# vidify/old-audiosync

Measured on NVIDIA B200. Metric: xcorr_pairs_per_sec_L1440000, higher is better.
Workload: dtype f32

## Files before the change

### old-audiosync_b200/csrc/fft_kernels.cuh

```cuda
#pragma once

#include "common.cuh"
#include "fft_device.cuh"

namespace asc {

constexpr int COL_T = 16;

constexpr int ctas_per_sm(size_t smem, int threads) {
    const int by_smem = (int)((228u * 1024u) / (smem + 1024u));
    const int by_threads = 1024 / threads;
    const int n = by_smem < by_threads ? by_smem : by_threads;
    return n >= 3 ? 3 : (n >= 1 ? n : 1);
}
constexpr unsigned TW2_BITS = 10;
constexpr unsigned TW2_MASK = (1u << TW2_BITS) - 1u;

template <class C>
ASC_HD C tw2(const C* __restrict__ lo, const C* __restrict__ hi, unsigned a) {
    return cmul(ldg(lo + (a & TW2_MASK)), ldg(hi + (a >> TW2_BITS)));
}

constexpr int tile_boxes(int rows) { return (rows + 255) / 256; }
constexpr int tile_box_rows(int rows) { return (rows + tile_boxes(rows) - 1) / tile_boxes(rows); }
constexpr int tile_box_start(int rows, int i) {
    return i * tile_box_rows(rows) + tile_box_rows(rows) <= rows ? i * tile_box_rows(rows) : rows - tile_box_rows(rows);
}

template <typename InT>
ASC_HD cplx load_packed(const InT* __restrict__ x, long long n, bool vec = true);

template <>
ASC_HD cplx load_packed<float>(const float* __restrict__ x, long long n, bool) {
    return ldg(reinterpret_cast<const float2*>(x) + n);
}
template <>
ASC_HD cplx load_packed<double>(const double* __restrict__ x, long long n, bool) {
    double2 d = ldg(reinterpret_cast<const double2*>(x) + n);
    return cmake(in_real<float>(d.x), in_real<float>(d.y));
}
template <>
ASC_HD cplx load_packed<int16_t>(const int16_t* __restrict__ x, long long n, bool vec) {
    if (vec) {
        const short2 s = ldg(reinterpret_cast<const short2*>(x) + n);
        return cmake(in_real<float>(s.x), in_real<float>(s.y));
    }
    return cmake(in_real<float>(ldg(x + 2 * n)), in_real<float>(ldg(x + 2 * n + 1)));
}

struct ArgmaxPair {
    unsigned long long best;
    float second;
};

struct ArgmaxAcc {
    unsigned long long best = 0ull;
    float second = 0.0f;
    float thr = 0.0f;
    ASC_HD void update(unsigned long long key, float a) {
        if (key > best) {
            if (best != 0ull && !argmax_key_is_seed(best)) second = fmaxf(second, argmax_key_mag(best));
            best = key;
        } else {
            second = fmaxf(second, a);
        }
        thr = fmaxf(thr, second);
    }
    ASC_HD void consider(float v, uint32_t index) {
        const float a = fabsf(v);
        if (a >= thr) update(argmax_key_abs(v, index), a);
    }
    ASC_HD void consider_seed(float v, PairPeak* pk) {
        update(argmax_key_seed(v), 0.0f);
        pk->seed_bits = float_order_bits(fabsf(v));
    }
    ASC_HD float best_mag() const { return best != 0ull && !argmax_key_is_seed(best) ? argmax_key_mag(best) : 0.0f; }
    ASC_HD ArgmaxPair result() const { ArgmaxPair r; r.best = best; r.second = second; return r; }
};

ASC_HD void argmax_merge(unsigned long long& best, float& second, unsigned long long ob, float os) {
    const unsigned long long lose = ob > best ? best : ob;
    best = ob > best ? ob : best;
    second = fmaxf(second, os);
    if (lose != 0ull && !argmax_key_is_seed(lose)) second = fmaxf(second, argmax_key_mag(lose));
}

template <class RL, int M2_, int NT, typename InT, bool TMA>
struct ColFwdKernel {
    static constexpr int M1 = RL::n;
    static constexpr int M2 = M2_;
    static constexpr int P = RL::count;
    static constexpr int THREADS = NT;
    static constexpr size_t SMEM = (size_t)M1 * COL_T * sizeof(cplx);
    static constexpr int MIN_CTAS = ctas_per_sm(SMEM, NT);
    static_assert(NT % COL_T == 0, "a thread must keep its column across items");
    static_assert(P >= 2, "column plans need at least two passes");
    static_assert(!TMA || std::is_same<InT, float>::value, "TMA staging copies packed fp32 pairs verbatim");
    static_assert(!TMA || M1 >= 4, "tile too small for a box");
    static_assert(M1 % 2 == 0, "the zero half of the sample must be whole tile rows");

    struct Params {
        const InT* sources;
        const InT* samples;
        cplx* planes;
        PairPeak* peaks;
        const cplx* tw;
        const cplx* tc;
        const cplx* m_lo;
        const cplx* m_hi;
        long long L;
        long long src_pitch;
        long long smp_pitch;
        int vec_src, vec_smp;
        CUtensorMap tm_src, tm_smp;
    };
    static constexpr int SRC_ROWS = M1 - 1, SMP_ROWS = M1 / 2;

    template <class Ex>
    static ASC_HD void run(Ex& ex, const Params& p, cplx* __restrict__ buf) {
        const int c0 = ex.bx() * COL_T;
        const int sig = ex.by();
        const long long pair = ex.bz();
        const long long M = p.L;
        const InT* __restrict__ x = sig == 0 ? p.sources + pair * (p.src_pitch ? p.src_pitch : 2 * M)
                                             : p.samples + pair * (p.smp_pitch ? p.smp_pitch : M);
        const long long nvalid = sig == 0 ? M : M / 2;
        [[maybe_unused]] const bool vec = sig == 0 ? p.vec_src != 0 : p.vec_smp != 0;
        cplx* __restrict__ out = p.planes + (pair * 2 + sig) * M;
        const bool clears_peak = ex.bx() == 0 && sig == 0;

        [[maybe_unused]] void* mbar = reinterpret_cast<char*>(buf) + SMEM - 8;
        if constexpr (TMA) {
            ex.phase([&](int tid) {
                if (tid == 0) {
                    if (clears_peak) p.peaks[pair] = cleared_peak();
                    mbar_init(mbar, 1);
                }
            });
            ex.phase([&](int tid) {
                if (tid == 0) {
                    const char* __restrict__ raw = reinterpret_cast<const char*>(x) + (size_t)c0 * sizeof(cplx);
                    constexpr size_t pitch = (size_t)M2 * sizeof(cplx);
                    if (sig == 0) {
                        constexpr int NB = tile_boxes(SRC_ROWS), BR = tile_box_rows(SRC_ROWS);
                        mbar_expect_tx(mbar, (unsigned)(NB * BR * 128));
                        static_for<0, NB>([&](auto I) {
                            constexpr int r0 = tile_box_start(SRC_ROWS, decltype(I)::value);
                            tma_load_rows(buf + r0 * COL_T, &p.tm_src, 2 * c0, r0, (int)pair, mbar, raw + r0 * pitch, pitch, BR);
                        });
                    } else {
                        constexpr int NB = tile_boxes(SMP_ROWS), BR = tile_box_rows(SMP_ROWS);
                        mbar_expect_tx(mbar, (unsigned)(NB * BR * 128));
                        static_for<0, NB>([&](auto I) {
                            constexpr int r0 = tile_box_start(SMP_ROWS, decltype(I)::value);
                            tma_load_rows(buf + r0 * COL_T, &p.tm_smp, 2 * c0, r0, (int)pair, mbar, raw + r0 * pitch, pitch, BR);
                        });
                    }
                }
                mbar_wait(mbar, 0);
            });
        }

        static_for<0, P>([&](auto PP) {
            constexpr int ps = decltype(PP)::value;
            constexpr int R = RL::r(ps);
            constexpr int S = RL::stride(ps);
            constexpr bool first = ps == 0, last = ps == P - 1;
            constexpr bool from_global = first && !TMA;
            constexpr int items = (M1 / R) * COL_T;
            ex.phase([&](int tid) {
                if (from_global && clears_peak && tid == 0) p.peaks[pair] = cleared_peak();
                const int c = tid & (COL_T - 1);
                if constexpr (!last) {
                    auto items_loop = [&](auto HZ) {
                        [[maybe_unused]] constexpr bool hz = decltype(HZ)::value;
                        cplx t[R];
                        for (int w = tid; w < items; w += NT) {
                            const int bf = w >> 4;
                            const int blk = (S * R == M1) ? 0 : bf / S;
                            const int j = bf - blk * S;
                            const int i0 = blk * (S * R) + j;
                            cplx v[R];
                            if constexpr (from_global) {
                                static_for<0, R>([&](auto Q) {
                                    constexpr int q = decltype(Q)::value;
                                    const long long n = (long long)(i0 + q * S) * M2 + c0 + c;
                                    v[q] = n < nvalid ? load_packed<InT>(x, n, vec) : cmake(0.f, 0.f);
                                });
                            } else {
                                static_for<0, R>([&](auto Q) {
                                    constexpr int q = decltype(Q)::value;
                                    if constexpr (hz && 2 * q >= R) {
                                        v[q] = cmake(0.f, 0.f);
                                    } else if constexpr (TMA && first && !hz && q == R - 1) {
                                        if (i0 == S - 1) v[q] = load_packed<InT>(x, (long long)(M1 - 1) * M2 + c0 + c);
                                        else v[q] = buf[(i0 + q * S) * COL_T + c];
                                    } else {
                                        v[q] = buf[(i0 + q * S) * COL_T + c];
                                    }
                                });
                                if constexpr (TMA && first) {
                                    if (i0 == S - 1 && c == COL_T - 1) mbar_inval(mbar);
                                }
                            }
                            dft_reg<R, -1>(v);
                            pass_twiddles<R>(p.tw + RL::tw_offset(ps), S, j, t);
                            buf[i0 * COL_T + c] = v[0];
                            static_for<1, R>([&](auto K) {
                                constexpr int k = decltype(K)::value;
                                buf[(i0 + k * S) * COL_T + c] = cmul(v[k], t[k]);
                            });
                        }
                    };
                    if constexpr (first && TMA) {
                        static_assert(R % 2 == 0 && S * R == M1, "zero-pad rows must be the inputs q >= R/2 of pass 0");
                        if (sig == 1) items_loop(std::true_type{});
                        else items_loop(std::false_type{});
                    } else {
                        items_loop(std::false_type{});
                    }
                } else {
                    constexpr int Wt = RL::weight(ps);
                    const unsigned n2 = (unsigned)(c0 + c);
                    constexpr bool lean_g = R > 8;
                    cplx g[R];
                    if constexpr (!lean_g) {
                        static_assert(R <= 8, "power chain written for k < 8");
                        g[1] = tw2(p.m_lo, p.m_hi, n2 * (unsigned)Wt);
                        static_for<2, R>([&](auto K) {
                            constexpr int k = decltype(K)::value;
                            g[k] = (k % 2 == 0) ? cmul(g[k / 2], g[k / 2]) : cmul(g[k - 1], g[1]);
                        });
                    } else {
                        static_for<1, R>([&](auto K) {
                            constexpr int k = decltype(K)::value;
                            if constexpr (!lean_g || (k & (k - 1)) == 0)
                                g[k] = tw2(p.m_lo, p.m_hi, n2 * (unsigned)(Wt * k));
                        });
                    }
                    constexpr int ITER = (items + NT - 1) / NT;
                    constexpr int CH = ITER <= 6 ? ITER : 4;
                    constexpr int DB = NT / COL_T, UNIT = RL::stride(0) / R;
                    constexpr bool STEP = ITER > 1 && DB % UNIT == 0;
                    constexpr int MSTEP = STEP ? DB / UNIT : 0;
                    [[maybe_unused]] int f0_run = 0;
                    [[maybe_unused]] cplx t0_run = cmake(1.f, 0.f), gstep = cmake(1.f, 0.f);
                    if constexpr (STEP) {
                        f0_run = RL::freq_of_pos(((tid < items ? tid : 0) >> 4) * R);
                        t0_run = cmul(ldg(p.tc + f0_run * COL_T + c), tw2(p.m_lo, p.m_hi, (unsigned)c0 * (unsigned)f0_run));
                        gstep = tw2(p.m_lo, p.m_hi, n2 * (unsigned)MSTEP);
                    }
                    for (int it0 = 0; it0 < ITER; it0 += CH) {
                        int f0s[CH];
                        cplx t0s[CH];
                        static_for<0, CH>([&](auto I) {
                            constexpr int i = decltype(I)::value;
                            if constexpr (STEP) {
                                f0s[i] = f0_run;
                                t0s[i] = t0_run;
                                f0_run += MSTEP;
                                t0_run = cmul(t0_run, gstep);
                            } else {
                                const int w = tid + (it0 + i) * NT;
                                f0s[i] = RL::freq_of_pos(((w < items ? w : 0) >> 4) * R);
                                t0s[i] = cmul(ldg(p.tc + f0s[i] * COL_T + c),
                                              tw2(p.m_lo, p.m_hi, (unsigned)c0 * (unsigned)f0s[i]));
                            }
                        });
                        static_for<0, CH>([&](auto I) {
                            constexpr int i = decltype(I)::value;
                            const int w = tid + (it0 + i) * NT;
                            if (w < items) {
                                const int i0 = (w >> 4) * R;
                                cplx v[R];
                                static_for<0, R>([&](auto Q) {
                                    constexpr int q = decltype(Q)::value;
                                    v[q] = buf[(i0 + q) * COL_T + c];
                                });
                                dft_reg<R, -1>(v);
                                const cplx t0 = t0s[i];
                                cplx* __restrict__ o = out + ((unsigned)f0s[i] * (unsigned)M2 + n2);
                                o[0] = cmul(v[0], t0);
                                static_for<1, R>([&](auto K) {
                                    constexpr int k = decltype(K)::value;
                                    cplx gk;
                                    if constexpr (!lean_g || (k & (k - 1)) == 0) {
                                        gk = g[k];
                                    } else {
                                        constexpr int hb = (k >= 16) ? 16 : (k >= 8) ? 8 : (k >= 4) ? 4 : 2;
                                        constexpr int rest = k - hb;
                                        if constexpr ((rest & (rest - 1)) == 0) {
                                            gk = cmul(g[hb], g[rest]);
                                        } else {
                                            constexpr int hb2 = (rest >= 8) ? 8 : (rest >= 4) ? 4 : 2;
                                            constexpr int rest2 = rest - hb2;
                                            static_assert(R <= 24, "k < 24: at most four one-bits, and then the last two are 2 + 1");
                                            if constexpr ((rest2 & (rest2 - 1)) == 0) gk = cmul(g[hb], cmul(g[hb2], g[rest2]));
                                            else gk = cmul(cmul(g[hb], g[hb2]), cmul(g[rest2 & ~1], g[1]));
                                        }
                                    }
                                    o[(size_t)k * Wt * M2] = cmul(v[k], cmul(t0, gk));
                                });
                            }
                        });
                    }
                }
            });
        });
    }
};

template <class RL, int M2_, int NT, bool TMA = true>
struct ColInvKernel {
    static_assert(TMA, "K_C's tiles are always staged by the TMA unit");
    static constexpr int M1 = RL::n;
    static constexpr int M2 = M2_;
    static constexpr int P = RL::count;
    static constexpr int THREADS = NT;
    static constexpr size_t SMEM = (size_t)M1 * COL_T * sizeof(cplx);
    static constexpr int MIN_CTAS = ctas_per_sm(SMEM, NT);
    static_assert(NT % COL_T == 0, "a thread must keep its column across items");
    static_assert(NT % 32 == 0, "the argmax epilogue votes per warp");
    static_assert(P >= 2, "column plans need at least two passes");

    struct Params {
        const cplx* planes;
        PairPeak* peaks;
        const cplx* tw;
        long long L;
        CUtensorMap tm;
    };
    static constexpr int TMA_ROWS = M1 - 1;

    template <class Ex>
    static ASC_HD void run(Ex& ex, const Params& p, cplx* __restrict__ buf) {
        const int c0 = ex.by() * COL_T;
        const long long pair = ex.bx();
        const long long M = p.L;
        const cplx* __restrict__ in = p.planes + pair * 2 * M;

        void* mbar = reinterpret_cast<char*>(buf) + SMEM - 8;
        ex.phase([&](int tid) {
            if (tid == 0) mbar_init(mbar, 1);
        });
        ex.phase([&](int tid) {
            if (tid == 0) {
                constexpr int NB = tile_boxes(TMA_ROWS), BR = tile_box_rows(TMA_ROWS);
                constexpr size_t pitch = (size_t)M2 * sizeof(cplx);
                const char* __restrict__ raw = reinterpret_cast<const char*>(in + c0);
                mbar_expect_tx(mbar, (unsigned)(NB * BR * 128));
                static_for<0, NB>([&](auto I) {
                    constexpr int r0 = tile_box_start(TMA_ROWS, decltype(I)::value);
                    tma_load_rows(buf + r0 * COL_T, &p.tm, 2 * c0, r0, (int)(2 * pair), mbar, raw + r0 * pitch, pitch, BR);
                });
            }
            mbar_wait(mbar, 0);
        });

        static_for<0, P - 1>([&](auto PP) {
            constexpr int ps = decltype(PP)::value;
            constexpr int R = RL::r(ps);
            constexpr int S = RL::stride(ps);
            constexpr int items = (M1 / R) * COL_T;
            ex.phase([&](int tid) {
                const int c = tid & (COL_T - 1);
                cplx t[R];
                for (int w = tid; w < items; w += NT) {
                    const int bf = w >> 4;
                    const int blk = (S * R == M1) ? 0 : bf / S;
                    const int j = bf - blk * S;
                    const int i0 = blk * (S * R) + j;
                    cplx v[R];
                    static_for<0, R>([&](auto Q) {
                        constexpr int q = decltype(Q)::value;
                        if constexpr (ps == 0 && q == R - 1) {
                            if (i0 == S - 1) v[q] = ldg(in + ((long long)(M1 - 1) * M2 + c0 + c));
                            else v[q] = buf[(i0 + q * S) * COL_T + c];
                        } else {
                            v[q] = buf[(i0 + q * S) * COL_T + c];
                        }
                    });
                    if constexpr (ps == 0) {
                        if (i0 == S - 1 && c == COL_T - 1) mbar_inval(mbar);
                    }
                    dft_reg<R, +1>(v);
                    pass_twiddles<R>(p.tw + RL::tw_offset(ps), S, j, t);
                    buf[i0 * COL_T + c] = v[0];
                    static_for<1, R>([&](auto K) {
                        constexpr int k = decltype(K)::value;
                        buf[(i0 + k * S) * COL_T + c] = cmulc(v[k], t[k]);
                    });
                }
            });
        });

        {
            constexpr int ps = P - 1;
            constexpr int R = RL::r(ps);
            constexpr int Wt = RL::weight(ps);
            constexpr int items = (M1 / R) * COL_T;
            ex.phase_argmax(
                [&](int tid) -> ArgmaxPair {
                    ArgmaxAcc acc;
                    const unsigned int seen = ex.peek_bits(&p.peaks[pair].second_bits);
                    if (seen != 0u) acc.thr = float_from_order_bits(seen);
                    const int c = tid & (COL_T - 1);
                    const bool col0 = (c0 + c) == 0;
                    for (int w0 = 0; w0 < items; w0 += NT) {
                        const int w = w0 + tid;
                        const bool act = w < items;
                        const int blk = (act ? w : 0) >> 4;
                        const int i0 = blk * R;
                        cplx v[R];
                        static_for<0, R>([&](auto Q) {
                            constexpr int q = decltype(Q)::value;
                            v[q] = buf[(i0 + q) * COL_T + c];
                        });
                        dft_reg<R, +1>(v);
                        float gm = fmaxf(fabsf(v[0].x), fabsf(v[0].y));
                        static_for<1, R>([&](auto K) {
                            constexpr int k = decltype(K)::value;
                            gm = fmaxf(gm, fmaxf(fabsf(v[k].x), fabsf(v[k].y)));
                        });
                        const bool has_seed = col0 && i0 == 0;
                        const bool need = act && (gm >= acc.thr || has_seed);
                        if (ex.any(need)) {
                            if (need) {
                                const int f0 = RL::freq_of_pos(i0);
                                static_for<0, R>([&](auto K) {
                                    constexpr int k = decltype(K)::value;
                                    const int n1 = f0 + k * Wt;
                                    const uint32_t i_re = 2u * ((uint32_t)n1 * (uint32_t)M2 + (uint32_t)(c0 + c));
                                    if (has_seed && n1 == 0) acc.consider_seed(v[k].x, &p.peaks[pair]);
                                    else acc.consider(v[k].x, i_re);
                                    acc.consider(v[k].y, i_re + 1u);
                                });
                            }
                            acc.thr = fmaxf(acc.thr, ex.warp_second(acc.best_mag(), acc.second));
                        }
                    }
                    return acc.result();
                },
                &p.peaks[pair].key, &p.peaks[pair].second_bits, buf);
        }
    }
};

ASC_HD void split_mul_merge(cplx a, cplx b, cplx c, cplx d, cplx w, cplx& qk, cplx& qmk) {
    const cplx s = cmake(a.x + b.x, a.y - b.y);
    const cplx t = cmake(a.x - b.x, a.y + b.y);
    const cplx u = cmul(w, cmake(t.y, -t.x));
    const cplx s2 = cmake(c.x + d.x, c.y - d.y);
    const cplx t2 = cmake(c.x - d.x, c.y + d.y);
    const cplx u2 = cmul(w, cmake(t2.y, -t2.x));
    const cplx p1 = cmulc(cadd(s, u), cadd(s2, u2));
    const cplx p2 = cmulc(csub(s, u), csub(s2, u2));
    const cplx g = cadd(p1, p2);
    const cplx e = csub(p1, p2);
    const cplx ce = cmulc(e, w);
    const cplx h = cmake(-ce.y, ce.x);
    qk = cmake(0.25f * (g.x + h.x), 0.25f * (g.y + h.y));
    qmk = cmake(0.25f * (g.x - h.x), -0.25f * (g.y - h.y));
}

template <class C>
ASC_HD void split_mul_merge_w2(C a, C b, C c, C d, C w2, C& qk2, C& qmk2) {
    const C s = cconj_add(a, b), t = cconj_sub(a, b);
    const C s2 = cconj_add(c, d), t2 = cconj_sub(c, d);
    const C g = cmulc_acc(t, t2, cmulc(s, s2));
    const C x = cmulc(s, t2);
    const C h = cmulc_nacc(x, w2, cmulc(t, s2));
    qk2 = cadd(g, h);
    const C e = csub(g, h);
    qmk2 = cmake(e.x, -e.y);
}

ASC_HD float phat_rsqrt(float q) {
#if defined(__CUDA_ARCH__)
    return rsqrtf(q);
#else
    return 1.0f / sqrtf(q);
#endif
}
ASC_HD double phat_rsqrt(double q) {
#if defined(__CUDA_ARCH__)
    return rsqrt(q);
#else
    return 1.0 / sqrt(q);
#endif
}
ASC_HD cplx unit_phasor(cplx z) {
    const float m = fmaxf(fabsf(z.x), fabsf(z.y));
    uint32_t b;
    memcpy(&b, &m, 4);
    int e = (int)(b >> 23);
    e = e < 1 ? 1 : (e > 253 ? 253 : e);
    const uint32_t sb = (uint32_t)(254 - e) << 23;
    float s;
    memcpy(&s, &sb, 4);
    const float x = z.x * s, y = z.y * s;
    const float q = fmaf(x, x, y * y);
    const float r = q > 0.0f ? phat_rsqrt(q) : 0.0f;
    return cmake(x * r, y * r);
}
ASC_HD cplxd unit_phasor(cplxd z) {
    const double m = fmax(fabs(z.x), fabs(z.y));
    uint64_t b;
    memcpy(&b, &m, 8);
    int e = (int)(b >> 52);
    e = e < 1 ? 1 : (e > 2045 ? 2045 : e);
    const uint64_t sb = (uint64_t)(2046 - e) << 52;
    double s;
    memcpy(&s, &sb, 8);
    const double x = z.x * s, y = z.y * s;
    const double q = fma(x, x, y * y);
    const double r = q > 0.0 ? phat_rsqrt(q) : 0.0;
    return cmake(x * r, y * r);
}

template <int SCALE, class C>
ASC_HD void split_phat_merge(C a, C b, C c, C d, C w, C& qk, C& qmk) {
    static_assert(SCALE == 1 || SCALE == 2, "output convention of split_mul_merge or split_mul_merge_w2");
    const C s = cconj_add(a, b), t = cconj_sub(a, b);
    const C s2 = cconj_add(c, d), t2 = cconj_sub(c, d);
    const C u = cmul_ni(cmul(w, t)), u2 = cmul_ni(cmul(w, t2));
    const C p1 = cmulc(unit_phasor(cadd(s, u)), unit_phasor(cadd(s2, u2)));
    const C p2 = cmulc(unit_phasor(csub(s, u)), unit_phasor(csub(s2, u2)));
    C g = cadd(p1, p2);
    C h = cmul_pi(cmulc(csub(p1, p2), w));
    if constexpr (SCALE == 2) {
        g = cadd(g, g);
        h = cadd(h, h);
    }
    qk = cadd(g, h);
    const C e = csub(g, h);
    qmk = cmake(e.x, -e.y);
}

template <class RL, int M1_, int NT, bool PHAT = false>
struct RowFusedKernel {
    static constexpr int M2 = RL::n;
    static constexpr int M1 = M1_;
    static constexpr int P = RL::count;
    static constexpr int THREADS = NT;
    static constexpr int RP = M2;
    static constexpr size_t SMEM = (size_t)4 * RP * sizeof(cplx);
    static constexpr int MIN_CTAS = ctas_per_sm(SMEM, NT);
    static constexpr int R0 = RL::r(0);
    static constexpr int S0 = RL::stride(0);
    static_assert(M2 % 2 == 0, "row length must be even (16-byte chunks, bulk store size)");
    static_assert(P >= 2, "row plans need at least two passes");
    static_assert(S0 * R0 == M2 && S0 >= 16, "pass 0 must own the last two points of a row as its last two items");

    static constexpr int slots(int S) { return (S > 1 && S < 16) ? 16 : S; }

    struct Params {
        cplx* planes;
        const cplx* tw;
        const cplx* rev;
        const cplx* m_lo;
        const cplx* m_hi;
        long long L;
        const cplx* rtab;
        int m1 = 0;
    };
    static constexpr int TABP = (S0 + R0 + 1) & ~1;
    static_assert(NT % 64 == 0, "the split phase maps threads to an (NT/64) x 64 grid");
    static constexpr int SPLIT_A = NT / 64;
    static constexpr int SPLIT_XN = (R0 + SPLIT_A - 1) / SPLIT_A;
    static constexpr int SPLIT_MN = (S0 + 63) / 64;
    static_assert(2 * TABP + 1 <= 2 * RP, "final-pass twiddle tables and their mbarrier must fit the dead sample rows");

    template <class Ex>
    static ASC_HD void run(Ex& ex, const Params& p, cplx* __restrict__ buf) {
        const int r = ex.bx();
        const long long pair = ex.bz();
        const long long M = p.L;
        const int m1 = M1 > 0 ? M1 : p.m1;
        const bool two = (r != 0) && (2 * r != m1);
        const int nrows = two ? 2 : 1;
        const int k1a = r, k1b = m1 - r;
        cplx* __restrict__ plane_s = p.planes + pair * 2 * M;
        cplx* __restrict__ plane_p = plane_s + M;
        cplx* __restrict__ tab = buf + 2 * RP;
        void* tabbar = buf + 2 * RP + 2 * TABP;

        {
            void* mbar = buf + 4 * RP - 1;
            ex.phase([&](int tid) {
                if (tid == 0) mbar_init(mbar, 1);
            });
            ex.phase([&](int tid) {
                if (tid == 0) {
                    constexpr unsigned full = (unsigned)(M2 * sizeof(cplx));
                    mbar_expect_tx(mbar, two ? 4u * full - 16u : 2u * full);
                    bulk_load(buf, plane_s + (long long)k1a * M2, full, mbar);
                    bulk_load(buf + 2 * RP, plane_p + (long long)k1a * M2, full, mbar);
                    if (two) {
                        bulk_load(buf + RP, plane_s + (long long)k1b * M2, full, mbar);
                        bulk_load(buf + 3 * RP, plane_p + (long long)k1b * M2, full - 16u, mbar);
                    }
                }
                mbar_wait(mbar, 0);
            });
        }

        auto fwd_pass = [&](auto PP, int t, int nt, int slot0, int sstep, int nb) {
            constexpr int ps = decltype(PP)::value;
            constexpr int R = RL::r(ps);
            constexpr int S = RL::stride(ps);
            constexpr int SL = slots(S);
            constexpr int per_row = (M2 / (S * R)) * SL;
            const int items = per_row * nb;
            [[maybe_unused]] const int tail_w = (slot0 + (nb - 1) * sstep == 3) ? items - 2 : 0x7fffffff;
            {
                for (int w = t; w < items; w += nt) {
                    const int bw = w / per_row;
                    const int bf = w - bw * per_row;
                    const int blk = (per_row == SL) ? 0 : bf / SL;
                    const int j = bf - blk * SL;
                    if (SL != S && j >= S) continue;
                    cplx* __restrict__ row = buf + (slot0 + bw * sstep) * RP;
                    const int i0 = blk * (S * R) + j;
                    cplx v[R];
                    static_for<0, R>([&](auto Q) {
                        constexpr int q = decltype(Q)::value;
                        v[q] = row[i0 + q * S];
                    });
                    if constexpr (ps == 0) {
                        if (w >= tail_w) {
                            v[R - 1] = ldg(plane_p + (long long)k1b * M2 + (i0 + (R - 1) * S));
                            if (w == tail_w + 1) mbar_inval(buf + 4 * RP - 1);
                        }
                    }
                    dft_reg<R, -1>(v);
                    row[i0] = v[0];
                    if constexpr (S > 1) {
                        cplx t[R];
                        pass_twiddles<R>(p.tw + RL::tw_offset(ps), S, j, t);
                        static_for<1, R>([&](auto K) {
                            constexpr int k = decltype(K)::value;
                            row[i0 + k * S] = cmul(v[k], t[k]);
                        });
                    } else {
                        static_for<1, R>([&](auto K) {
                            constexpr int k = decltype(K)::value;
                            row[i0 + k] = v[k];
                        });
                    }
                }
            }
        };
        static_for<0, P>([&](auto PP) {
            ex.phase([&](int tid) { fwd_pass(PP, tid, NT, 0, two ? 1 : 2, 2 * nrows); });
        });

        {
            ex.phase([&](int tid) {
                const cplx wk1 = tw2(p.m_lo, p.m_hi, (unsigned)k1a);
                if (two) {
                    cplx* __restrict__ zs_a = buf;
                    cplx* __restrict__ zs_b = buf + RP;
                    cplx* __restrict__ zp_a = buf + 2 * RP;
                    cplx* __restrict__ zp_b = buf + 3 * RP;
                    cplx ax[SPLIT_XN], cm[SPLIT_MN];
                    const int sa = tid >> 6, sb = tid & 63;
                    static_for<0, SPLIT_XN>([&](auto X) {
                        const int d0 = sa + decltype(X)::value * SPLIT_A;
                        ax[decltype(X)::value] = cmul(ldg(p.rev + (d0 < R0 ? d0 : 0) * S0), wk1);
                    });
                    static_for<0, SPLIT_MN>([&](auto Mm) {
                        const int e1 = sb + decltype(Mm)::value * 64;
                        cm[decltype(Mm)::value] = ldg(p.rev + (e1 < S0 ? e1 : 0));
                    });
                    static_for<0, SPLIT_MN>([&](auto Mm) {
#if defined(__CUDA_ARCH__)
                        if constexpr (decltype(Mm)::value > 0 && decltype(Mm)::value % 2 == 0)
                            asm volatile("" ::: "memory");
#endif
                        static_for<0, SPLIT_XN>([&](auto X) {
                            const int d0 = sa + decltype(X)::value * SPLIT_A;
                            const int e1 = sb + decltype(Mm)::value * 64;
                            if (d0 < R0 && e1 < S0) {
                                const int e = d0 * S0 + e1;
                                const int pb = M2 - 1 - e;
                                const cplx w2 = cmul(ax[decltype(X)::value], cm[decltype(Mm)::value]);
                                cplx qk, qmk;
                                if constexpr (PHAT) split_phat_merge<2>(zs_a[e], zs_b[pb], zp_a[e], zp_b[pb], w2, qk, qmk);
                                else split_mul_merge_w2(zs_a[e], zs_b[pb], zp_a[e], zp_b[pb], w2, qk, qmk);
                                zs_a[e] = qk;
                                zs_b[pb] = qmk;
                            }
                        });
                    });
                } else {
                    cplx* __restrict__ zs = buf;
                    cplx* __restrict__ zp = buf + 2 * RP;
                    const int items = r == 0 ? M2 / 2 + 1 : M2 / 2;
                    for (int e = tid; e < items; e += NT) {
                        int pa, pb;
                        if (r == 0) {
                            pa = RL::pos_of_freq(e);
                            pb = RL::pos_of_freq(e == 0 ? 0 : M2 - e);
                        } else {
                            pa = e;
                            pb = M2 - 1 - e;
                        }
                        const cplx w2 = cmul(ldg(p.rev + pa), wk1);
                        cplx qk, qmk;
                        if constexpr (PHAT) split_phat_merge<2>(zs[pa], zs[pb], zp[pa], zp[pb], w2, qk, qmk);
                        else split_mul_merge_w2(zs[pa], zs[pb], zp[pa], zp[pb], w2, qk, qmk);
                        zs[pa] = qk;
                        if (pa != pb) zs[pb] = qmk;
                    }
                }
            });
        }

        ex.single([&]() {
            constexpr unsigned bytes = (unsigned)(TABP * sizeof(cplx));
            mbar_init(tabbar, 1);
            mbar_expect_tx(tabbar, (unsigned)nrows * bytes);
            bulk_load(tab, p.rtab + (long long)k1a * TABP, bytes, tabbar);
            if (two) bulk_load(tab + TABP, p.rtab + (long long)k1b * TABP, bytes, tabbar);
        });

        auto inv_pass = [&](auto PP, int t, int nt, int r0, int nr) {
            constexpr int ps = P - 1 - decltype(PP)::value;
            constexpr int R = RL::r(ps);
            constexpr int S = RL::stride(ps);
            constexpr int SL = slots(S);
            constexpr bool last = ps == 0;
            constexpr int per_row = (M2 / (S * R)) * SL;
            const int items = per_row * nr;
            {
                if constexpr (last) mbar_wait(tabbar, 0);
                for (int w = t; w < items; w += nt) {
                    const int rw = w / per_row;
                    const int rr = r0 + rw;
                    const int bf = w - rw * per_row;
                    const int blk = (per_row == SL) ? 0 : bf / SL;
                    const int j = bf - blk * SL;
                    if (SL != S && j >= S) continue;
                    cplx* __restrict__ row = buf + rr * RP;
                    const int i0 = blk * (S * R) + j;
                    cplx v[R];
                    v[0] = row[i0];
                    if constexpr (S > 1) {
                        cplx t[R];
                        pass_twiddles<R>(p.tw + RL::tw_offset(ps), S, j, t);
                        static_for<1, R>([&](auto Q) {
                            constexpr int q = decltype(Q)::value;
                            v[q] = cmulc(row[i0 + q * S], t[q]);
                        });
                    } else {
                        static_for<1, R>([&](auto Q) {
                            constexpr int q = decltype(Q)::value;
                            v[q] = row[i0 + q];
                        });
                    }
                    dft_reg<R, +1>(v);
                    if constexpr (!last) {
                        static_for<0, R>([&](auto K) {
                            constexpr int k = decltype(K)::value;
                            row[i0 + k * S] = v[k];
                        });
                    } else {
                        const cplx t0 = tab[rr * TABP + j];
                        row[j] = cmulc(v[0], t0);
                        static_for<1, R>([&](auto K) {
                            constexpr int k = decltype(K)::value;
                            row[j + k * S] = cmulc(v[k], cmul(t0, tab[rr * TABP + S0 + k]));
                        });
                    }
                }
                if constexpr (last) fence_async_proxy();
            }
        };
        static_for<0, P>([&](auto PP) {
            ex.phase([&](int tid) { inv_pass(PP, tid, NT, 0, nrows); });
        });

        ex.single([&]() {
            bulk_store(plane_s + (long long)k1a * M2, buf, (unsigned)(M2 * sizeof(cplx)));
            if (two) bulk_store(plane_s + (long long)k1b * M2, buf + RP, (unsigned)(M2 * sizeof(cplx)));
            bulk_store_commit_and_drain();
        });
    }
};

struct DeviceExec {
    int x_ = 0, y_ = 0, z_ = 0;
    ASC_HD int bx() const { return x_; }
    ASC_HD int by() const { return y_; }
    ASC_HD int bz() const { return z_; }
    template <class F>
    ASC_HD void phase(F&& f) {
#if defined(__CUDA_ARCH__)
        f((int)threadIdx.x);
        __syncthreads();
#endif
    }
    template <class F>
    ASC_HD void single(F&& f) {
#if defined(__CUDA_ARCH__)
        if (threadIdx.x == 0) f();
#endif
    }
    ASC_HD bool any(bool b) const {
#if defined(__CUDA_ARCH__)
        return __any_sync(0xffffffffu, b);
#else
        return b;
#endif
    }
    ASC_HD float warp_second(float best_mag, float second) const {
#if defined(__CUDA_ARCH__)
        const unsigned bm = __float_as_uint(fmaxf(best_mag, 0.0f));
        const unsigned top = __reduce_max_sync(0xffffffffu, bm);
        const unsigned holders = __ballot_sync(0xffffffffu, bm == top);
        const bool winner = (threadIdx.x & 31u) == (unsigned)(__ffs(holders) - 1);
        const float cand = winner ? second : fmaxf(second, best_mag);
        return __uint_as_float(__reduce_max_sync(0xffffffffu, __float_as_uint(fmaxf(cand, 0.0f))));
#else
        (void)best_mag;
        return second;
#endif
    }
    ASC_HD unsigned long long peek_key(const unsigned long long* k) const {
#if defined(__CUDA_ARCH__)
        return __ldcg(k);
#else
        return *k;
#endif
    }
    ASC_HD unsigned int peek_bits(const unsigned int* k) const {
#if defined(__CUDA_ARCH__)
        return __ldcg(k);
#else
        return *k;
#endif
    }
    template <class F>
    ASC_HD void phase_argmax(F&& f, unsigned long long* dst, unsigned int* dst_second, void* scratch) {
#if defined(__CUDA_ARCH__)
        unsigned long long* s_best = reinterpret_cast<unsigned long long*>(scratch);
        float* s_sec = reinterpret_cast<float*>(s_best + 32);
        const ArgmaxPair mine = f((int)threadIdx.x);
        unsigned long long best = mine.best;
        float second = mine.second;
        for (int o = 16; o > 0; o >>= 1)
            argmax_merge(best, second, __shfl_xor_sync(0xffffffffu, best, o), __shfl_xor_sync(0xffffffffu, second, o));
        const int wid = threadIdx.x >> 5, lane = threadIdx.x & 31;
        const int nw = (blockDim.x + 31) >> 5;
        __syncthreads();
        if (lane == 0) { s_best[wid] = best; s_sec[wid] = second; }
        __syncthreads();
        if (wid == 0) {
            best = lane < nw ? s_best[lane] : 0ull;
            second = lane < nw ? s_sec[lane] : 0.0f;
            for (int o = 16; o > 0; o >>= 1)
                argmax_merge(best, second, __shfl_xor_sync(0xffffffffu, best, o), __shfl_xor_sync(0xffffffffu, second, o));
            if (lane == 0) {
                const unsigned long long old = atomicMax(dst, best);
                if (old != best) argmax_merge(best, second, old, 0.0f);
                atomicMax(dst_second, float_order_bits(second));
            }
        }
#endif
    }
};

#if defined(__CUDACC__)
template <class K, class = void>
struct min_ctas_of { static constexpr int value = 1; };
template <class K>
struct min_ctas_of<K, std::void_t<decltype(K::MIN_CTAS)>> { static constexpr int value = K::MIN_CTAS; };

template <class K>
__global__ void __launch_bounds__(K::THREADS, min_ctas_of<K>::value)
fft_kernel_entry(const __grid_constant__ typename K::Params p) {
    extern __shared__ __align__(128) unsigned char asc_smem[];
    pdl_prologue();
    DeviceExec ex;
    ex.x_ = (int)blockIdx.x; ex.y_ = (int)blockIdx.y; ex.z_ = (int)blockIdx.z;
    K::run(ex, p, reinterpret_cast<cplx*>(asc_smem));
}
#endif

}
```

Baseline: 42820.

## Stage the product-plane spectra in Blackwell tensor memory across the split and merge phase

For the 2400-point row configuration, the last forward pass writes the product-plane 15-point butterfly outputs for 128 blocks per row into tensor memory using tcgen05.st instead of shared memory. The split/merge phase then reads those values back with tcgen05.ld, and the first inverse pass reads them again, so part of the shared-memory traffic and bank pressure is moved to TMEM. The change adds TMEM allocation and deallocation, tcgen05 fences around each barrier, and a custom mapping of threads to TMEM lanes. The remaining blocks still go through the shared-memory path, which makes the work distribution uneven across threads and adds complexity.

```diff
diff --git a/old-audiosync_b200/csrc/fft_kernels.cuh b/old-audiosync_b200/csrc/fft_kernels.cuh
--- a/old-audiosync_b200/csrc/fft_kernels.cuh
+++ b/old-audiosync_b200/csrc/fft_kernels.cuh
@@ -1,4 +1,7 @@
 #pragma once
+
+#include <cstdio>
+#include <cstdlib>
 
 #include "common.cuh"
 #include "fft_device.cuh"
@@ -537,6 +540,123 @@
     qmk = cmake(e.x, -e.y);
 }
 
+constexpr int ROW_TM_COLS = 64;
+ASC_HD int tm_own_lane(int tid) { return 32 * ((tid >> 5) & 3) + (tid & 31); }
+#if !defined(__CUDA_ARCH__)
+inline float* host_tmem() {
+    static thread_local float cells[128 * ROW_TM_COLS];
+    return cells;
+}
+inline void host_tm_check(int tid, int lane, int col, int words) {
+    if (lane != tm_own_lane(tid) || col < 0 || col + words > ROW_TM_COLS) {
+        fprintf(stderr, "tensor memory: thread %d cannot reach lane %d, columns %d..%d\n", tid, lane, col, col + words - 1);
+        abort();
+    }
+}
+#endif
+template <int N>
+ASC_HD void tm_st(uint32_t tbase, int tid, int lane, int col, const cplx* v) {
+#if defined(__CUDA_ARCH__)
+    (void)tid;
+    uint32_t a = tbase + ((uint32_t)(lane & ~31) << 16) + (uint32_t)col;
+    const uint32_t* r = reinterpret_cast<const uint32_t*>(v);
+    int w = 0;
+    if constexpr (2 * N >= 16) {
+        asm volatile("tcgen05.st.sync.aligned.32x32b.x16.b32 [%0], {%1,%2,%3,%4,%5,%6,%7,%8,%9,%10,%11,%12,%13,%14,%15,%16};"
+            :: "r"(a), "r"(r[0]), "r"(r[1]), "r"(r[2]), "r"(r[3]), "r"(r[4]), "r"(r[5]), "r"(r[6]), "r"(r[7]),
+               "r"(r[8]), "r"(r[9]), "r"(r[10]), "r"(r[11]), "r"(r[12]), "r"(r[13]), "r"(r[14]), "r"(r[15]) : "memory");
+        w = 16;
+    }
+    if constexpr ((2 * N) & 8) {
+        asm volatile("tcgen05.st.sync.aligned.32x32b.x8.b32 [%0], {%1,%2,%3,%4,%5,%6,%7,%8};"
+            :: "r"(a + w), "r"(r[w]), "r"(r[w + 1]), "r"(r[w + 2]), "r"(r[w + 3]), "r"(r[w + 4]), "r"(r[w + 5]),
+               "r"(r[w + 6]), "r"(r[w + 7]) : "memory");
+        w += 8;
+    }
+    if constexpr ((2 * N) & 4) {
+        asm volatile("tcgen05.st.sync.aligned.32x32b.x4.b32 [%0], {%1,%2,%3,%4};"
+            :: "r"(a + w), "r"(r[w]), "r"(r[w + 1]), "r"(r[w + 2]), "r"(r[w + 3]) : "memory");
+        w += 4;
+    }
+    if constexpr ((2 * N) & 2) {
+        asm volatile("tcgen05.st.sync.aligned.32x32b.x2.b32 [%0], {%1,%2};" :: "r"(a + w), "r"(r[w]), "r"(r[w + 1]) : "memory");
+    }
+    static_assert(2 * N < 32, "at most 15 complex values per access");
+#else
+    (void)tbase;
+    host_tm_check(tid, lane, col, 2 * N);
+    memcpy(host_tmem() + lane * ROW_TM_COLS + col, v, N * sizeof(cplx));
+#endif
+}
+template <int N>
+ASC_HD void tm_ld(uint32_t tbase, int tid, int lane, int col, cplx* v) {
+#if defined(__CUDA_ARCH__)
+    (void)tid;
+    uint32_t a = tbase + ((uint32_t)(lane & ~31) << 16) + (uint32_t)col;
+    uint32_t* r = reinterpret_cast<uint32_t*>(v);
+    int w = 0;
+    if constexpr (2 * N >= 16) {
+        asm volatile("tcgen05.ld.sync.aligned.32x32b.x16.b32 {%0,%1,%2,%3,%4,%5,%6,%7,%8,%9,%10,%11,%12,%13,%14,%15}, [%16];"
+            : "=r"(r[0]), "=r"(r[1]), "=r"(r[2]), "=r"(r[3]), "=r"(r[4]), "=r"(r[5]), "=r"(r[6]), "=r"(r[7]),
+              "=r"(r[8]), "=r"(r[9]), "=r"(r[10]), "=r"(r[11]), "=r"(r[12]), "=r"(r[13]), "=r"(r[14]), "=r"(r[15])
+            : "r"(a) : "memory");
+        w = 16;
+    }
+    if constexpr ((2 * N) & 8) {
+        asm volatile("tcgen05.ld.sync.aligned.32x32b.x8.b32 {%0,%1,%2,%3,%4,%5,%6,%7}, [%8];"
+            : "=r"(r[w]), "=r"(r[w + 1]), "=r"(r[w + 2]), "=r"(r[w + 3]), "=r"(r[w + 4]), "=r"(r[w + 5]),
+              "=r"(r[w + 6]), "=r"(r[w + 7]) : "r"(a + w) : "memory");
+        w += 8;
+    }
+    if constexpr ((2 * N) & 4) {
+        asm volatile("tcgen05.ld.sync.aligned.32x32b.x4.b32 {%0,%1,%2,%3}, [%4];"
+            : "=r"(r[w]), "=r"(r[w + 1]), "=r"(r[w + 2]), "=r"(r[w + 3]) : "r"(a + w) : "memory");
+        w += 4;
+    }
+    if constexpr ((2 * N) & 2) {
+        asm volatile("tcgen05.ld.sync.aligned.32x32b.x2.b32 {%0,%1}, [%2];" : "=r"(r[w]), "=r"(r[w + 1]) : "r"(a + w) : "memory");
+    }
+    static_assert(2 * N < 32, "at most 15 complex values per access");
+#else
+    (void)tbase;
+    host_tm_check(tid, lane, col, 2 * N);
+    memcpy(v, host_tmem() + lane * ROW_TM_COLS + col, N * sizeof(cplx));
+#endif
+}
+ASC_HD void tm_wait_ld() {
+#if defined(__CUDA_ARCH__)
+    asm volatile("tcgen05.wait::ld.sync.aligned;" ::: "memory");
+#endif
+}
+ASC_HD void tm_before_barrier() {
+#if defined(__CUDA_ARCH__)
+    asm volatile("tcgen05.wait::st.sync.aligned;" ::: "memory");
+    asm volatile("tcgen05.fence::before_thread_sync;" ::: "memory");
+#endif
+}
+ASC_HD void tm_after_barrier() {
+#if defined(__CUDA_ARCH__)
+    asm volatile("tcgen05.fence::after_thread_sync;" ::: "memory");
+#endif
+}
+ASC_HD void tm_alloc(void* dst) {
+#if defined(__CUDA_ARCH__)
+    asm volatile("tcgen05.alloc.cta_group::1.sync.aligned.shared::cta.b32 [%0], %1;"
+                 :: "r"((uint32_t)__cvta_generic_to_shared(dst)), "n"(ROW_TM_COLS) : "memory");
+    asm volatile("tcgen05.relinquish_alloc_permit.cta_group::1.sync.aligned;" ::: "memory");
+    asm volatile("tcgen05.fence::before_thread_sync;" ::: "memory");
+#else
+    (void)dst;
+#endif
+}
+ASC_HD void tm_dealloc(uint32_t tbase) {
+#if defined(__CUDA_ARCH__)
+    asm volatile("tcgen05.dealloc.cta_group::1.sync.aligned.b32 %0, %1;" :: "r"(tbase), "n"(ROW_TM_COLS) : "memory");
+#else
+    (void)tbase;
+#endif
+}
+
 template <class RL, int M1_, int NT, bool PHAT = false>
 struct RowFusedKernel {
     static constexpr int M2 = RL::n;
@@ -571,6 +691,13 @@
     static constexpr int SPLIT_MN = (S0 + 63) / 64;
     static_assert(2 * TABP + 1 <= 2 * RP, "final-pass twiddle tables and their mbarrier must fit the dead sample rows");
 
+    static constexpr bool TM = M2 == 2400 && NT == 320 && S0 == 240 && RL::r(P - 1) == 15 && RL::stride(P - 1) == 1;
+    static constexpr int TM_QUADS = 128;
+    static ASC_HD int tm_quad_of_lane(int lane) {
+        const int l = lane & 31;
+        return 4 * (lane >> 5) + (l >> 3) + 16 * (l & 7);
+    }
+
     template <class Ex>
     static ASC_HD void run(Ex& ex, const Params& p, cplx* __restrict__ buf) {
         const int r = ex.bx();
@@ -582,6 +709,7 @@
         const int k1a = r, k1b = m1 - r;
         cplx* __restrict__ plane_s = p.planes + pair * 2 * M;
         cplx* __restrict__ plane_p = plane_s + M;
+        [[maybe_unused]] uint32_t tbase = 0;
         cplx* __restrict__ tab = buf + 2 * RP;
         void* tabbar = buf + 2 * RP + 2 * TABP;
 
@@ -589,6 +717,9 @@
             void* mbar = buf + 4 * RP - 1;
             ex.phase([&](int tid) {
                 if (tid == 0) mbar_init(mbar, 1);
+                if constexpr (TM) {
+                    if (two && (tid >> 5) == 0) tm_alloc(buf + 4 * RP - 2);
+                }
             });
             ex.phase([&](int tid) {
                 if (tid == 0) {
@@ -602,6 +733,12 @@
                     }
                 }
                 mbar_wait(mbar, 0);
+                if constexpr (TM) {
+                    if (two) {
+                        tm_after_barrier();
+                        tbase = *reinterpret_cast<const uint32_t*>(buf + 4 * RP - 2);
+                    }
+                }
             });
         }
 
@@ -652,13 +789,93 @@
             }
         };
         static_for<0, P>([&](auto PP) {
-            ex.phase([&](int tid) { fwd_pass(PP, tid, NT, 0, two ? 1 : 2, 2 * nrows); });
+            if constexpr (TM && decltype(PP)::value == P - 1) {
+                ex.phase([&](int tid) {
+                    if (!two) { fwd_pass(PP, tid, NT, 0, 2, 2); return; }
+                    constexpr int R = 15, NB = M2 / R;
+                    auto bfly = [&](int slot, int blk, cplx (&v)[R]) {
+                        const cplx* row = buf + slot * RP + blk * R;
+                        static_for<0, R>([&](auto Q) { v[decltype(Q)::value] = row[decltype(Q)::value]; });
+                        dft_reg<R, -1>(v);
+                    };
+                    if (tid < 2 * TM_QUADS) {
+                        const int lane = tm_own_lane(tid), hi = tid >> 7;
+                        const int b = tm_quad_of_lane(lane);
+                        cplx v[R];
+                        bfly(2 + hi, hi ? NB - 1 - b : b, v);
+                        tm_st<R>(tbase, tid, lane, hi ? 2 * R : 0, v);
+                        tm_before_barrier();
+                    }
+                    for (int k = tid; k < 2 * NB + 2 * (NB - TM_QUADS); k += NT - 2 * TM_QUADS) {
+                        int slot, blk;
+                        if (k < 2 * NB) { slot = k / NB; blk = k - slot * NB; }
+                        else if (k < 2 * NB + (NB - TM_QUADS)) { slot = 2; blk = TM_QUADS + (k - 2 * NB); }
+                        else { slot = 3; blk = k - 2 * NB - (NB - TM_QUADS); }
+                        cplx v[R];
+                        bfly(slot, blk, v);
+                        cplx* row = buf + slot * RP + blk * R;
+                        static_for<0, R>([&](auto K) { row[decltype(K)::value] = v[decltype(K)::value]; });
+                        if (tid < 2 * TM_QUADS) break;
+                    }
+                });
+            } else {
+                ex.phase([&](int tid) { fwd_pass(PP, tid, NT, 0, two ? 1 : 2, 2 * nrows); });
+            }
         });
 
         {
             ex.phase([&](int tid) {
                 const cplx wk1 = tw2(p.m_lo, p.m_hi, (unsigned)k1a);
-                if (two) {
+                if (TM && two) {
+                    cplx* __restrict__ zs_a = buf;
+                    cplx* __restrict__ zs_b = buf + RP;
+                    tm_after_barrier();
+                    const int lane = tm_own_lane(tid), g = tid >> 7, q = (tid >> 5) & 3;
+                    const int b = tm_quad_of_lane(lane);
+                    const cplx ax = cmul(ldg(p.rev + (b >> 4) * S0), wk1);
+                    const cplx* __restrict__ cm = p.rev + 15 * (b & 15);
+                    auto chunk = [&](auto CC, int i0) {
+                        constexpr int C = decltype(CC)::value;
+                        cplx za[C], zb[C];
+                        tm_ld<C>(tbase, tid, lane, 2 * i0, za);
+                        tm_ld<C>(tbase, tid, lane, 30 + 2 * (14 - (i0 + C - 1)), zb);
+                        tm_wait_ld();
+                        cplx qa[C], qb[C];
+                        static_for<0, C>([&](auto J) {
+                            constexpr int j = decltype(J)::value;
+                            const int e = 15 * b + i0 + j;
+                            const int pb = M2 - 1 - e;
+                            const cplx w2 = cmul(ax, ldg(cm + i0 + j));
+                            if constexpr (PHAT) split_phat_merge<2>(zs_a[e], zs_b[pb], za[j], zb[C - 1 - j], w2, qa[j], qb[C - 1 - j]);
+                            else split_mul_merge_w2(zs_a[e], zs_b[pb], za[j], zb[C - 1 - j], w2, qa[j], qb[C - 1 - j]);
+                        });
+                        tm_st<C>(tbase, tid, lane, 2 * i0, qa);
+                        tm_st<C>(tbase, tid, lane, 30 + 2 * (14 - (i0 + C - 1)), qb);
+                    };
+                    constexpr int CH = PHAT ? 2 : 4;
+                    int i = q >= 2 ? 8 * g : 5 * g;
+                    int n = q >= 2 ? 8 - g : 5;
+                    for (; n >= CH; n -= CH, i += CH) chunk(std::integral_constant<int, CH>{}, i);
+                    if (n & 2) { chunk(std::integral_constant<int, 2>{}, i); i += 2; }
+                    if (n & 1) chunk(std::integral_constant<int, 1>{}, i);
+                    if (q < 2) {
+                        cplx* __restrict__ zp_a = buf + 2 * RP;
+                        cplx* __restrict__ zp_b = buf + 3 * RP;
+                        const int r6 = (2 * g + q) * 32 + (tid & 31);
+                        for (int sidx = r6; sidx < 15 * (M2 / 15 - TM_QUADS); sidx += 192) {
+                            const int e = 15 * TM_QUADS + sidx;
+                            const int pb = M2 - 1 - e;
+                            const int d0 = e / S0;
+                            const cplx w2 = cmul(cmul(ldg(p.rev + d0 * S0), wk1), ldg(p.rev + (e - d0 * S0)));
+                            cplx qk, qmk;
+                            if constexpr (PHAT) split_phat_merge<2>(zs_a[e], zs_b[pb], zp_a[e], zp_b[pb], w2, qk, qmk);
+                            else split_mul_merge_w2(zs_a[e], zs_b[pb], zp_a[e], zp_b[pb], w2, qk, qmk);
+                            zs_a[e] = qk;
+                            zs_b[pb] = qmk;
+                        }
+                    }
+                    tm_before_barrier();
+                } else if (two) {
                     cplx* __restrict__ zs_a = buf;
                     cplx* __restrict__ zs_b = buf + RP;
                     cplx* __restrict__ zp_a = buf + 2 * RP;
@@ -778,7 +995,40 @@
             }
         };
         static_for<0, P>([&](auto PP) {
-            ex.phase([&](int tid) { inv_pass(PP, tid, NT, 0, nrows); });
+            if constexpr (TM && decltype(PP)::value == 0) {
+                ex.phase([&](int tid) {
+                    if (!two) { inv_pass(PP, tid, NT, 0, nrows); return; }
+                    constexpr int R = 15, NB = M2 / R;
+                    cplx v[R];
+                    int slot, blk;
+                    if (tid < 2 * TM_QUADS) {
+                        tm_after_barrier();
+                        const int lane = tm_own_lane(tid);
+                        const int b = tm_quad_of_lane(lane);
+                        slot = tid >> 7;
+                        blk = slot ? NB - 1 - b : b;
+                        tm_ld<R>(tbase, tid, lane, slot ? 2 * R : 0, v);
+                        tm_wait_ld();
+                        tm_before_barrier();
+                    } else {
+                        const int u = tid - 2 * TM_QUADS;
+                        slot = u < NB - TM_QUADS ? 0 : 1;
+                        blk = slot ? u - (NB - TM_QUADS) : TM_QUADS + u;
+                        const cplx* row = buf + slot * RP + blk * R;
+                        static_for<0, R>([&](auto Q) { v[decltype(Q)::value] = row[decltype(Q)::value]; });
+                    }
+                    dft_reg<R, +1>(v);
+                    cplx* row = buf + slot * RP + blk * R;
+                    static_for<0, R>([&](auto K) { row[decltype(K)::value] = v[decltype(K)::value]; });
+                });
+            } else {
+                ex.phase([&](int tid) {
+                    if constexpr (TM && decltype(PP)::value == 1) {
+                        if (two && (tid >> 5) == 0) { tm_after_barrier(); tm_dealloc(tbase); }
+                    }
+                    inv_pass(PP, tid, NT, 0, nrows);
+                });
+            }
         });
 
         ex.single([&]() {
```

New measurement: 38400, median of 6. 10.3% lower.
